# dan-lee-gh/monte-carlo-gp

Measured on AMD Instinct MI355X. Metric: race-simulations/sec (20 drivers, 60 laps), higher is better.
Workload: dtype f64

## Files before the change

monte_carlo_gp_amd/csrc/race_kernel_reg.hip.h:

```cpp
#pragma once
#include "race_common.hip.h"
#include "race_isa.hip.h"
#include "sort_networks.h"

#include <utility>

#ifndef MCGP_STAT
#define MCGP_STAT(what, value)
#endif
#ifndef MCGP_TRACE_PASS
#define MCGP_TRACE_PASS(sim, lap, pass, n_cand)
#endif
#ifndef MCGP_COOPERATIVE_EVENTS
#define MCGP_COOPERATIVE_EVENTS 1
#endif
#ifndef MCGP_GRID_EXACT
#define MCGP_GRID_EXACT 0
#endif
#ifndef MCGP_WIDE_EXACT
#define MCGP_WIDE_EXACT 0
#endif
#ifndef MCGP_WIDE_TIE_SHIFT
#define MCGP_WIDE_TIE_SHIFT 0
#endif

namespace mcgp {

constexpr uint32_t k3UsedMask = 7u;
constexpr uint32_t k3Drs = 1u << 3;
constexpr int k3IdShift = 4;
constexpr uint32_t k3IdMask = 31u << k3IdShift;
constexpr uint32_t k3Dnf = 1u << 9;
constexpr uint32_t k3SlotMask = k3IdMask | k3Dnf;
constexpr int k3CompShift = 10;
constexpr uint32_t k3CompMask = 7u << k3CompShift;
constexpr uint32_t k3Dirty = 1u << 13;
constexpr int k3AgeShift = 16;
constexpr uint32_t k3AgeMask = 0x7FFu << k3AgeShift;
constexpr int k3GposShift = 27;
__host__ __device__ constexpr uint32_t pk_driver16(uint32_t p) { return p & k3IdMask; }
__host__ __device__ constexpr uint32_t pk_slot16(uint32_t p) { return p & k3SlotMask; }
__host__ __device__ constexpr uint32_t pk_comp512(uint32_t p) { return (p & k3CompMask) >> (k3CompShift - 9); }
__host__ __device__ constexpr uint32_t pk_comp16(uint32_t p) { return (p >> (k3CompShift - 4)) & 0x70u; }
constexpr double kAgeFieldUnit = 1.0 / 65536.0;

constexpr size_t kLdsPerCu = 160 * 1024;
__host__ __device__ constexpr size_t align16(size_t x) { return (x + 15) / 16 * 16; }
constexpr int kWordRows = 8;
__host__ __device__ constexpr size_t per_thread_lds_bytes_reg(int n) { return (size_t)kWordRows * 4 + (size_t)n * 8; }
constexpr int kNumCompounds = 5;
__host__ __device__ constexpr size_t shared_lds_bytes_reg(int n)
{
    return (size_t)kNormalRows * 16 + (size_t)n * 16 + (size_t)(kMaxCars + n) * 16 +
           (size_t)((kNumCompounds - 1) * kMaxCars + n) * 16 + kCompStride * 16 + 64 + 128 + align16((size_t)n * n * 4) +
           align16((size_t)n * n * 8);
}
__host__ __device__ constexpr int reg_min_waves(int n) { return n <= 6 ? (n == 4 ? 4 : 6) : n <= 11 ? 4 : n <= 22 ? 3 : 2; }
constexpr int kMaxBlockWaves = 16;
constexpr size_t kLdsReserve = 256;
__host__ __device__ constexpr int block_shape_rank(int w) { return (w % 4 == 0 ? 0 : 100) + (w <= 8 ? 2 * (8 - w) : w - 8); }
__host__ __device__ constexpr int reg_block_waves(int n)
{
    const int cap = 4 * reg_min_waves(n);
    int best = 0, waves = 1;
    for (int w = 1; w <= kMaxBlockWaves; ++w) {
        int b = (int)((kLdsPerCu - kLdsReserve) / (shared_lds_bytes_reg(n) + (size_t)w * 64 * per_thread_lds_bytes_reg(n)));
        if (b * w > cap) b = cap / w;
        if (b < 1) continue;
        if (b * w > best || (b * w == best && block_shape_rank(w) < block_shape_rank(waves))) { best = b * w; waves = w; }
    }
    return waves;
}

__host__ __device__ constexpr size_t reg_retire_ws_bytes(int n, size_t lanes) { return (size_t)(n + 1) * lanes * 4; }

constexpr int kWideLdsRowsMax = 32 * 16;
constexpr int kNorm53LdsStride = 80;
__host__ __device__ constexpr size_t wide_fixed_lds_bytes(int n, int waves)
{
    return shared_lds_bytes_reg(n) - (size_t)kNormalRows * 16 + (size_t)waves * 64 * per_thread_lds_bytes_reg(n);
}
__host__ __device__ constexpr int wide_lds_rows(int n, int waves)
{
    const size_t fixed = wide_fixed_lds_bytes(n, waves);
    const size_t room = kLdsPerCu - kLdsReserve > fixed ? kLdsPerCu - kLdsReserve - fixed : 0;
    int rows = (int)(room / (size_t)kNorm53LdsStride) / 16 * 16;
    return rows > kWideLdsRowsMax ? kWideLdsRowsMax : rows;
}
__host__ __device__ constexpr size_t wide_lds_bytes(int n, int waves)
{
    return wide_fixed_lds_bytes(n, waves) + (size_t)wide_lds_rows(n, waves) * kNorm53LdsStride;
}
__host__ __device__ constexpr size_t wide_chain_bytes(int n, int total_laps)
{
    return total_laps >= 2 ? (size_t)(total_laps - 1) * (size_t)((n + 3) & ~3) * 8 : 0;
}
__host__ __device__ constexpr size_t wide_launch_lds_bytes(int n, int waves, int total_laps)
{
    const size_t base = wide_lds_bytes(n, waves), chain = wide_chain_bytes(n, total_laps);
    return base + chain + kLdsReserve <= kLdsPerCu ? base + chain : base;
}
template <int N, int WAVES = reg_block_waves(N), bool WIDE = false>
struct RegGeo {
    static constexpr int kWaves = WAVES;
    static constexpr bool kWide = WIDE;
    static constexpr int B = 64 * kWaves;
    static constexpr uint32_t oDrvA = 0;
    static constexpr uint32_t oDrvB = oDrvA + N * 16;
    static constexpr uint32_t oIc = oDrvB + (kMaxCars + N) * 16;
    static constexpr uint32_t oComp = oIc + ((kNumCompounds - 1) * kMaxCars + N) * 16;
    static constexpr uint32_t oDrs = oComp + kCompStride * 16;
    static constexpr uint32_t oPit = oDrs + 16;
    static constexpr uint32_t oDrsB = oDrs + 32;
    static constexpr uint32_t oLut = oDrsB + 32;
    static constexpr uint32_t oNorm = oLut + 128;
    static constexpr uint32_t oHist = oNorm + (WIDE ? 0 : kNormalRows * 16);
    static_assert(WIDE || oNorm >= kNormalRowBias * 16, "the inverse-normal rows are addressed through a base 48 rows before the table");
    static constexpr uint32_t oGrid = oHist + (uint32_t)align16((size_t)N * N * 4);
    static constexpr uint32_t oW = oGrid + (uint32_t)align16((size_t)N * N * 8);
    static constexpr uint32_t oLast = oW + (uint32_t)kWordRows * B * 4;
    static constexpr uint32_t oNorm53 = oLast + (uint32_t)N * B * 8;
    static constexpr int kNorm53Rows = WIDE ? wide_lds_rows(N, WAVES) : 0;
    static constexpr int kNorm53First = kNormal53Rows - kNorm53Rows;
    static constexpr uint32_t kBytes = oNorm53 + (uint32_t)kNorm53Rows * (uint32_t)kNorm53LdsStride;
    static constexpr uint32_t oChain = kBytes;
    static constexpr uint32_t kChainStride = (uint32_t)((N + 3) & ~3) * 8u;
    __host__ __device__ static constexpr bool chain_fits(int total_laps)
    {
        return WIDE && total_laps >= 2 && kBytes + wide_chain_bytes(N, total_laps) + kLdsReserve <= kLdsPerCu;
    }
    static_assert(oW == shared_lds_bytes_reg(N) - (WIDE ? (size_t)kNormalRows * 16 : 0) && oLast % 8 == 0, "LDS map");
    static_assert(oW % 16 == 0 && oNorm53 % 16 == 0, "the event handler parks fields with 16-byte LDS accesses (ds_write_b128 / ds_read_b128); table rows are read 16 bytes at a time");
    static_assert(kBytes == (WIDE ? wide_lds_bytes(N, WAVES) : per_thread_lds_bytes_reg(N) * B + shared_lds_bytes_reg(N)), "LDS map");
    static_assert(kBytes + kLdsReserve <= kLdsPerCu, "block does not fit LDS");
    static_assert(oLast < 65536, "row bases must fit the DS immediate offset");
};
constexpr int kWideMinLdsRows = 14 * 16;
__host__ __device__ constexpr int wide_block_waves(int n)
{
    if (n <= 22) {
        for (int w = 12; w > 8; --w)
            if (wide_fixed_lds_bytes(n, w) + kLdsReserve <= kLdsPerCu && wide_lds_rows(n, w) >= kWideMinLdsRows) return w;
    }
    int w = 8;
    while (w > 1 && wide_fixed_lds_bytes(n, w) + kLdsReserve > kLdsPerCu) --w;
    return w;
}
__host__ __device__ constexpr int wide_min_waves(int n) { return wide_block_waves(n) > 8 ? 3 : 2; }
template <int N>
using WideGeo = RegGeo<N, wide_block_waves(N), true>;

template <int N>
struct SortNetwork {
    int a[N * 8];
    int b[N * 8];
    int step[N * 8];
    int n;
    int ga[N * 8];
    int gn[N * 8];
    int n_groups;
    constexpr SortNetwork() : a{}, b{}, step{}, n(0), ga{}, gn{}, n_groups(0)
    {
        const SortNetworkTable *table = nullptr;
        for (const SortNetworkTable &t : kSortNetworks)
            if (t.n == N) table = &t;
        if (table) {
            for (int i = 0; i < table->size; ++i) {
                a[n] = table->pairs[i][0];
                b[n] = table->pairs[i][1];
                step[n] = table->pairs[i][2];
                ++n;
            }
        } else {
            int t = 0, s = 0;
            while ((1 << t) < N) ++t;
            for (int p = t > 0 ? 1 << (t - 1) : 0; p > 0; p >>= 1) {
                int q = 1 << (t - 1), r = 0, d = p;
                while (true) {
                    for (int i = 0; i < N - d; ++i)
                        if ((i & p) == r) { a[n] = i; b[n] = i + d; step[n] = s; ++n; }
                    ++s;
                    if (q == p) break;
                    d = q - p;
                    q >>= 1;
                    r = p;
                }
            }
        }
        for (int i = 0; i < n;) {
            const int len = (i + 1 < n && step[i + 1] == step[i]) ? 2 : 1;
            ga[n_groups] = i;
            gn[n_groups] = len;
            ++n_groups;
            i += len;
        }
    }
};

__device__ __forceinline__ bool cmpx(double &ca, uint32_t &pa, double &cb, uint32_t &pb)
{
    const bool sw = (ca > cb) || (ca == cb && pa > pb);
    double c0, c1;
// ... 146 lines not shown
    return strict;
}

template <int N, bool DISTINCT = false>
__device__ __forceinline__ void update_positions_reg(const double (&cum)[N], uint32_t (&pk)[N],
                                                     bool drs_allowed, double dirty_thr)
{
    bool first = true;
    double leader = 0.0, prev = 0.0;
#pragma unroll
    for (int i = 0; i < N; ++i) {
        const uint32_t p = pk[i];
        const bool act = !(p & k3Dnf);
        const double t = cum[i];
        leader = (act && first) ? t : leader;
        const double tbl = t - leader;
        const bool dirty = (DISTINCT ? !first : tbl > 0) && tbl < dirty_thr;
        const bool drs = !first && drs_allowed && (t - prev) < 1.0;
        pk[i] = (p & ~(k3Drs | k3Dirty)) | (dirty ? k3Dirty : 0u) | (drs ? k3Drs : 0u);
        prev = act ? t : prev;
        first = first && !act;
    }
}

__host__ __device__ constexpr int pit_regime(int remaining_laps)
{
    return remaining_laps > 30 ? 0 : remaining_laps > 20 ? 1 : remaining_laps > 15 ? 2 : 3;
}
__device__ __forceinline__ uint32_t pit_rule_word(int track, int regime, uint32_t used, uint32_t pop_sh, uint32_t pop_mh)
{
    const int remaining_laps = regime == 0 ? 31 : regime == 1 ? 21 : regime == 2 ? 16 : 0;
    uint32_t newc = stint_compound(track, remaining_laps);
    if (track == 0 && __popc(used) == 1 && ((used >> newc) & 1u)) {
        const uint32_t avail = 7u & ~used;
        const uint32_t popped = avail == 5u ? pop_sh : avail == 6u ? pop_mh : 0u;
        if (remaining_laps > 20) newc = (avail & 2u) ? 1u : popped;
        else newc = (avail & 1u) ? 0u : popped;
    }
    return (newc << k3CompShift) | ((used | (1u << newc)) & k3UsedMask);
}

constexpr double kRegTimeFloor = 8.0;
__host__ __device__ inline double reg_time_floor(const KParams &kp)
{
    const double z_max = kp.wide ? 8.5 : 6.5;
    double floor_ = __builtin_inf();
    double cdelta_min = __builtin_inf();
    for (int c = 0; c < 5; ++c) cdelta_min = kp.comp_delta[c] < cdelta_min ? kp.comp_delta[c] : cdelta_min;
    for (int d = 0; d < kp.n; ++d) {
        double eff_min = 0.0;
        for (int c = 0; c < 5; ++c) {
            const double e = kp.comp_deg[c] * kp.factor[d];
            eff_min = e < eff_min ? e : eff_min;
        }
        const double var = kp.variance[d] < 0 ? -kp.variance[d] : kp.variance[d];
        const double f = kp.base_pace[d] - var * z_max + eff_min * 2047.0;
        floor_ = f < floor_ ? f : floor_;
        if (!(f == f)) return f;
    }
    floor_ = floor_ + cdelta_min - 110.0 * 0.03 - (kp.drs_delta > 0 ? kp.drs_delta : 0.0) +
             (kp.dirty_pen < 0 ? kp.dirty_pen : 0.0) - 0.5 * 1.5 * z_max;
    return floor_;
}

__host__ __device__ inline bool reg_kernel_serves(const KParams &kp)
{
    if (!(kp.overtake_delta >= 0.0)) return false;
    const double big = 0x1p900, tiny = 0x1p-900;
    auto scalable = [&](double x) { return x == 0.0 || (x > -big && x < big && (x >= tiny || x <= -tiny)); };
    for (int d = 0; d < kp.n; ++d) {
        if (!scalable(kp.base_pace[d]) || !scalable(kp.tire_deg[d])) return false;
        for (int c = 0; c < 5; ++c)
            if (!scalable(kp.comp_deg[c] * kp.factor[d])) return false;
    }
    return reg_time_floor(kp) >= kRegTimeFloor;
}

template <int N, class G = RegGeo<N>>
__device__ __forceinline__ void reg_load_tables(const KParams *__restrict__ P, unsigned char *smem, uint32_t tid,
                                                const double *__restrict__ norm53 = nullptr)
{
    constexpr int B = G::B;
    uint32_t *s_hist = reinterpret_cast<uint32_t *>(smem + G::oHist);
    double *t_grid = reinterpret_cast<double *>(smem + G::oGrid);
    if constexpr (G::kWide) {
        double *t53 = reinterpret_cast<double *>(smem + G::oNorm53);
        for (uint32_t i = tid; i < (uint32_t)G::kNorm53Rows * 8u; i += B)
            t53[(i >> 3) * (kNorm53LdsStride / 8) + (i & 7u)] = norm53[(uint32_t)G::kNorm53First * 8u + i];
        if (G::chain_fits(P->total_laps)) {
            for (uint32_t d = tid; d < G::kChainStride / 8u; d += B) {
                const uint64_t q = d < (uint32_t)N ? P->q64_dnf[d] : 0ull;
                uint64_t S = q;
                for (int k = 2; k <= P->total_laps; ++k) {
                    *reinterpret_cast<uint64_t *>(smem + G::oChain + (uint32_t)(k - 2) * G::kChainStride + d * 8u) = S;
                    S = __umul64hi(S, q);
                }
            }
        }
    } else {
        float4 *t_norm = reinterpret_cast<float4 *>(smem + G::oNorm);
        for (uint32_t i = tid; i < (uint32_t)kNormalRows * 4; i += B)
            reinterpret_cast<uint32_t *>(t_norm)[i] = P->normal_bits[i];
    }
    for (uint32_t d = tid; d < (uint32_t)N; d += B) {
        double *a = reinterpret_cast<double *>(smem + G::oDrvA + d * 16);
        double *b = reinterpret_cast<double *>(smem + G::oDrvB + d * 16);
        const double qnan = __builtin_nan("");
        a[0] = P->variance[d];
        a[1] = P->base_pace[d];
        b[0] = P->base_pace[d] * 2147483648.0;
        b[1] = P->tire_deg[d] * 32768.0;
        b[2 * kMaxCars] = qnan;
        b[2 * kMaxCars + 1] = qnan;
    }
    if (tid < 2) {
        *reinterpret_cast<double *>(smem + G::oDrs + tid * k3Drs) = tid ? P->drs_delta : 0.0;
        *reinterpret_cast<double *>(smem + G::oDrsB + tid * k3Drs) = tid ? P->drs_delta * 2147483648.0 : 0.0;
        *reinterpret_cast<double *>(smem + G::oPit + tid * 8u) = tid ? P->pit_loss : 0.0;
    }
    for (uint32_t i = tid; i < (uint32_t)kNumCompounds * N; i += B) {
        const uint32_t c = i / N, d = i % N;
        unsigned char *r = smem + G::oIc + (c * kMaxCars + d) * 16;
        *reinterpret_cast<double *>(r) = (P->comp_deg[c] * P->factor[d]) * kAgeFieldUnit;
        *reinterpret_cast<uint32_t *>(r + 8) = (uint32_t)P->opt_laps[d * kCompStride + c] << 16;
        *reinterpret_cast<uint32_t *>(r + 12) = 0u;
    }
    for (uint32_t i = tid; i < 32u; i += B)
        *reinterpret_cast<uint32_t *>(smem + G::oLut + i * 4) =
            pit_rule_word(P->track, (int)(i >> 3), i & 7u, (uint32_t)P->pop_sh, (uint32_t)P->pop_mh);
    for (uint32_t c = tid; c < (uint32_t)kCompStride; c += B) {
        double *r = reinterpret_cast<double *>(smem + G::oComp + c * 16);
        r[0] = P->comp_delta[c];
        r[1] = 0.0;
    }
    for (uint32_t i = tid; i < (uint32_t)(N * N); i += B) {
        s_hist[i] = 0u;
        t_grid[(i % N) * N + (i / N)] = P->grid_probs[i];
    }
}

template <int N, class G = RegGeo<N>>
__device__ __forceinline__ void reg_flush_hist(unsigned char *smem, uint32_t tid, unsigned long long *__restrict__ hist)
{
    const uint32_t *s_hist = reinterpret_cast<const uint32_t *>(smem + G::oHist);
    for (uint32_t i = tid; i < (uint32_t)(N * N); i += G::B) {
        const uint32_t c = s_hist[i];
        if (c) atomicAdd(&hist[i], (unsigned long long)c);
    }
}

__device__ __forceinline__ uint32_t uniform_u32(uint32_t x)
{
#if defined(__HIP_DEVICE_COMPILE__)
    return (uint32_t)__builtin_amdgcn_readfirstlane((int)x);
#else
    return x;
#endif
}
template <int N, class G>
__device__ __forceinline__ uint32_t wide_pass_exact_body(const uint32_t (&pk)[N], double od31, uint32_t lap, uint32_t pass, uint32_t c0l,
                                                         uint32_t c1l, uint32_t k0l, uint32_t k1l, uint32_t tid)
{
    constexpr int B = G::B;
    const uint32_t tid4 = tid * 4u;
    auto w_row_ = [&](int r) -> uint32_t { return G::oW + (uint32_t)r * (B * 4) + tid4; };
    uint32_t hits53 = 0u;
    uint64_t thr64[N];
    uint32_t cand = 0u;
    {
        double pace_prev = 0.0;
#pragma unroll
        for (int i = 0; i < N; ++i) {
            const f64x2 bd = lds_ld_f64x2(G::oDrvB + pk_slot16(pk[i]));
            const double pace = bd.x + (double)(pk[i] & k3AgeMask) * bd.y;
            thr64[i] = 0ull;
            if (i > 0) {
                const double dl = (pace_prev - pace) + lds_ld<double>(G::oDrsB + (pk[i] & k3Drs));
                const bool c = dl > od31;
                double x = ceil_f64(dl * 0x1p21);
                x = x < 0x1p52 ? x : 0x1p52;
                const uint32_t xh = c ? cvt_u32_f64_sat(x * 0x1p-32) : 0u;
                const uint32_t xl = c ? cvt_u32_f64_sat(x - (double)xh * 0x1p32) : 0u;
                thr64[i] = ((uint64_t)xh << 32) | (uint64_t)xl;
                cand |= c ? (1u << i) : 0u;
            }
            pace_prev = pace;
        }
    }
    uint32_t rest = cand;
#pragma unroll 1
    for (int chunk = 0; MCGP_ANY(rest != 0u); ++chunk) {
        uint32_t m = rest;
#pragma unroll 1
        for (int k = 0; k < 4 && m != 0u; ++k) m &= m - 1u;
        const uint32_t cur = rest & ~m;
        uint32_t o0, o1, o2, o3;
        philox4x32_10(c0l, c1l, (uint32_t)lap, kPurposeOvt | (uint32_t)(8 * pass + chunk), k0l, k1l, o0, o1, o2, o3);
        lds_st<uint32_t>(w_row_(0), o0);
        lds_st<uint32_t>(w_row_(1), o1);
        lds_st<uint32_t>(w_row_(2), o2);
        lds_st<uint32_t>(w_row_(3), o3);
        philox4x32_10(c0l, c1l, (uint32_t)lap, kPurposeOvt | kCompanion | (uint32_t)(8 * pass + chunk), k0l, k1l, o0, o1, o2, o3);
        lds_st<uint32_t>(w_row_(4), o0);
        lds_st<uint32_t>(w_row_(5), o1);
        lds_st<uint32_t>(w_row_(6), o2);
        lds_st<uint32_t>(w_row_(7), o3);
        uint32_t h = 0u;
#pragma unroll
        for (int i = 1; i < N; ++i) {
            const uint32_t r = (uint32_t)__popc(cur & ((1u << i) - 1u)) * (uint32_t)(B * 4) + tid4;
            const uint64_t u = uniform53(lds_ld<uint32_t>(G::oW + r), lds_ld<uint32_t>(G::oW + (uint32_t)(4 * B * 4) + r));
            h |= u < thr64[i] ? (1u << i) : 0u;
        }
        hits53 |= h & cur;
        rest = m;
    }
    return hits53;
}
template <int N>
struct PkWords {
    uint32_t v[N];
};
template <int N, class G>
__device__ __attribute__((noinline)) uint32_t wide_pass_exact_fn(PkWords<N> field, double od31, uint32_t lap, uint32_t pass, uint32_t c0l,
                                                                 uint32_t c1l, uint32_t k0l_, uint32_t k1l_, uint32_t tid)
{
    return wide_pass_exact_body<N, G>(field.v, od31, lap, pass, c0l, c1l, uniform_u32(k0l_), uniform_u32(k1l_), tid);
}

template <int N, bool WIDE = false, class G = RegGeo<N>>
__device__ __forceinline__ void reg_simulate(const KParams *__restrict__ P, unsigned char *smem, uint32_t tid,
                                             uint32_t *__restrict__ ticket, uint64_t n_sims,
                                             uint64_t sim_offset, uint32_t seed_lo, uint32_t seed_hi,
                                             uint8_t *__restrict__ orders, const uint8_t *__restrict__ fixed_grid,
                                             uint32_t n_chunks, uint32_t *__restrict__ retire_ws_base, uint32_t ws_stride,
                                             uint32_t ws_first_lane, const double *__restrict__ norm53 = nullptr)
{
    constexpr int B = G::B;
    constexpr int kStepBatch = 4;
    constexpr bool kLean = WIDE && wide_min_waves(N) >= 3;
    constexpr int kPaceBatch = 5;
    static_assert(kStepBatch % 4 == 0, "a Philox block serves four consecutive places");
    const uint32_t tid4 = tid * 4u, tid8 = tid * 8u;
    const int L = P->total_laps;
    const int track = P->track;

    uint32_t *s_hist = reinterpret_cast<uint32_t *>(smem + G::oHist);

    auto w_row = [&](int r) -> uint32_t { return G::oW + (uint32_t)r * (B * 4) + tid4; };
    auto l_row = [&](int d) -> uint32_t { return G::oLast + (uint32_t)d * (B * 8) + tid8; };
    auto last_of = [&](uint32_t p) -> uint32_t { return ((p >> k3IdShift) & 31u) * (uint32_t)(B * 8) + tid8; };
    auto grid_byte = [&](int pos) -> uint32_t { return G::oW + (uint32_t)(pos >> 2) * (B * 4) + tid4 + (uint32_t)(pos & 3); };
    auto norm_row = [&](uint32_t off) -> float4 { return lds_ld_float4(G::oNorm - kNormalRowBias * 16u + off); };
    constexpr uint32_t kRareHi = (kNormal53HiBias + (uint32_t)(G::kNorm53First > 16 ? G::kNorm53First : 16)) << 16;
    [[maybe_unused]] auto norm53_row = [&](uint32_t hi, double (&c)[8]) {
        const uint32_t a = (hi >> 16) * (uint32_t)kNorm53LdsStride + (G::oNorm53 - (kNormal53HiBias + (uint32_t)G::kNorm53First) * (uint32_t)kNorm53LdsStride);
#pragma unroll
        for (int k = 0; k < 4; ++k) {
            const f64x2 v = lds_ld_f64x2(a + 16u * k);
            c[2 * k] = v.x;
            c[2 * k + 1] = v.y;
        }
    };
    [[maybe_unused]] auto normal53_one = [&](uint32_t w, uint32_t x) -> double {
        uint32_t hi;
        double t;
        normal53_prepare(w, x, hi, t);
        if (__builtin_expect(MCGP_ANY(G::kNorm53Rows == 0 || MCGP_WIDE_EXACT || hi < kRareHi), 0)) return normal53(w, x, norm53);
        double c[8];
        norm53_row(hi, c);
        return normal53_evaluate(w, c, t);
    };

    const double dirty_thr = P->dirty_thr;
    const float kNaN = __uint_as_float(0x7fc00000u);

    struct SlotIn {
        uint32_t pitw;
        double last, var, base, eff, cdelta, drs;
        uint32_t la;
        uint32_t fit;
    };
    auto load_slot = [&](uint32_t p, uint32_t lut_base) -> SlotIn {
        SlotIn r;
        r.fit = lds_ld<uint32_t>(((p & k3UsedMask) << 2) + lut_base);
        const uint32_t id16 = pk_driver16(p);
        r.la = id16 * (uint32_t)(B / 2) + tid8;
        r.last = lds_ld<double>(G::oLast + r.la);
        const uint32_t ic = id16 + pk_comp512(p);
        const f64x2 vb = lds_ld_f64x2(G::oDrvA + id16);
        r.var = vb.x;
        r.base = vb.y;
        uint32_t pad;
        lds_ld_f64_u32x2(G::oIc + ic, r.eff, r.pitw, pad);
        r.cdelta = lds_ld<double>(G::oComp + pk_comp16(p));
        r.drs = lds_ld<double>(G::oDrs + (p & k3Drs));
        return r;
    };

    for (uint32_t turn = 0u;; ++turn) {
        const uint32_t chunk = next_ticket(ticket, tid, turn, G::kWaves);
        if (chunk >= n_chunks) break;
        const uint64_t local = (uint64_t)chunk * 64ull + (uint64_t)(tid & 63u);
        const bool live = local < n_sims;
        if (!MCGP_ANY(live)) continue;
        const uint64_t sim = sim_offset + local;
        const uint32_t c0 = (uint32_t)sim, c1 = (uint32_t)(sim >> 32);

        double cum[N];
        uint32_t pk[N];

        {
            uint32_t remaining = (N >= 32) ? 0xffffffffu : ((1u << N) - 1u);
            int n_remaining = N;
            uint32_t g0 = 0, g1 = 0, g2 = 0, g3 = 0, h0 = 0, h1 = 0, h2 = 0, h3 = 0;
#pragma unroll 1
            for (int pos = 0; pos < N; ++pos) {
                uint32_t sel;
                if (fixed_grid) {
                    sel = fixed_grid[pos];
                } else {
                    if ((pos & 3) == 0) {
                        philox4x32_10(c0, c1, 0u, kPurposeGrid | (uint32_t)(pos >> 2), seed_lo, seed_hi, g0, g1, g2, g3);
                        if constexpr (WIDE)
                            philox4x32_10(c0, c1, 0u, kPurposeGrid | kCompanion | (uint32_t)(pos >> 2), seed_lo, seed_hi, h0, h1, h2, h3);
                    }
                    const uint32_t gw = (pos & 3) == 0 ? g0 : (pos & 3) == 1 ? g1 : (pos & 3) == 2 ? g2 : g3;
                    const uint32_t hw = (pos & 3) == 0 ? h0 : (pos & 3) == 1 ? h1 : (pos & 3) == 2 ? h2 : h3;
                    const double u = WIDE ? (double)uniform53(gw, hw) * 0x1p-53 : u32_to_unit(gw);
                    const uint32_t gcol = G::oGrid + (uint32_t)(pos * N) * 8u;
                    double acc = 0.0;
                    double A[N];
#pragma unroll
                    for (int d = 0; d < N; ++d) {
                        const double pd = ((remaining >> d) & 1u) ? lds_ld<double>(gcol + 8u * d) : 0.0;
                        acc = acc + pd;
                        A[d] = acc;
                    }
                    const double total = acc;
                    const double uc = u * total;
                    const double sure_gt = uc * (1.0 + 0x1p-40), sure_le = uc * (1.0 - 0x1p-40);
                    uint32_t n_le = 0u, n_le_lo = 0u;
#pragma unroll
                    for (int d = 0; d < N; ++d) {
                        n_le += A[d] > sure_gt ? 0u : 1u;
                        n_le_lo += A[d] > sure_le ? 0u : 1u;
                    }
                    const bool exact_path = MCGP_GRID_EXACT || !(total > 0x1p-900 && total < 0x1p900) || n_le != n_le_lo || n_le >= (uint32_t)N;
                    sel = n_le;
                    if (__builtin_expect(MCGP_ANY(exact_path), 0)) {
                        double p[N];
#pragma unroll
                        for (int d = 0; d < N; ++d) p[d] = ((remaining >> d) & 1u) ? lds_ld<double>(gcol + 8u * d) : 0.0;
                        const bool has_mass = total > 0;
                        const double uniform_p = 1.0 / (double)n_remaining;
                        double prob_sum = 0.0;
#pragma unroll
                        for (int d = 0; d < N; ++d) {
                            const double q = has_mass ? p[d] / total : uniform_p;
                            p[d] = ((remaining >> d) & 1u) ? q : 0.0;
                            prob_sum = prob_sum + p[d];
                        }
                        if (prob_sum > 0 && fabs(prob_sum - 1.0) > 1e-9) {
#pragma unroll
                            for (int d = 0; d < N; ++d) p[d] = p[d] / prob_sum;
                        }
                        double cdf = 0.0;
#pragma unroll
                        for (int d = 0; d < N; ++d) {
                            cdf = cdf + p[d];
                            p[d] = cdf;
                        }
                        const double cdf_last = cdf;
                        uint32_t above = 0u;
#pragma unroll
                        for (int d = 0; d < N; ++d) above |= !(p[d] / cdf_last <= u) ? (1u << d) : 0u;
                        const uint32_t sel_exact = above ? (uint32_t)__ffs((int)above) - 1u : 31u - (uint32_t)__clz((int)remaining);
                        sel = exact_path ? sel_exact : sel;
                    }
                }
                if ((remaining >> sel) & 1u) { remaining &= ~(1u << sel); --n_remaining; }
                lds_st<uint8_t>(grid_byte(pos), (uint8_t)sel);
            }
        }

#pragma unroll
        for (int i = 0; i < N; ++i) {
            const uint32_t id = lds_ld<uint8_t>(grid_byte(i));
            uint32_t comp, age;
            if (track == 2) { comp = 4u; age = 0u; }
            else if (track == 1) { comp = 3u; age = 0u; }
            else { comp = i < 10 ? 0u : 1u; age = i < 10 ? 4u : 0u; }
            pk[i] = (age << k3AgeShift) | (comp << k3CompShift) | ((1u << comp) & k3UsedMask) | (id << k3IdShift) |
                    ((uint32_t)i << k3GposShift);
            cum[i] = 0.0;
        }

        if constexpr (WIDE) {
#pragma unroll 1
            for (int d = 0; d < N; ++d) {
                uint32_t w0, w1, w2, w3, x0, x1, x2, x3;
                philox4x32_10(c0, c1, 1u, kPurposeCar | (uint32_t)d, seed_lo, seed_hi, w0, w1, w2, w3);
                philox4x32_10(c0, c1, 1u, kPurposeCar | kCompanion | (uint32_t)d, seed_lo, seed_hi, x0, x1, x2, x3);
                const bool out = uniform53(w0, x0) < P->t53_dnf1[d];
                lds_st<double>(l_row(d), out ? __builtin_nan("") : normal53_one(w1, x1));
            }
#pragma unroll
            for (int i = 0; i < N; ++i) {
                const uint32_t p = pk[i];
                const double z = lds_ld<double>(G::oLast + last_of(p));
                const uint32_t id16 = pk_driver16(p);
                const f64x2 vb = lds_ld_f64x2(G::oDrvA + id16);
                const double eff = lds_ld<double>(G::oIc + id16 + pk_comp512(p));
                const double cdelta = lds_ld<double>(G::oComp + pk_comp16(p));
                if (z != z) {
                    pk[i] = (p & ~k3AgeMask) | k3Dnf | (1u << k3AgeShift);
                    cum[i] = -(double)(i + 1) * 0x1p-1000;
                } else {
                    const double tire = (double)(p & k3AgeMask) * eff;
                    const double fuel_effect = (110.0 - 110.0) * 0.03;
                    const double noise = 0.0 + vb.x * z;
                    cum[i] = vb.y + tire - fuel_effect + cdelta - 0.0 + noise;
                }
            }
#pragma unroll 1
            for (int d = 0; d < N; ++d) {
                uint32_t w0, w1, w2, w3, x0, x1, x2, x3;
                philox4x32_10(c0, c1, 1u, kPurposeCar | (uint32_t)d, seed_lo, seed_hi, w0, w1, w2, w3);
                philox4x32_10(c0, c1, 1u, kPurposeCar | kCompanion | (uint32_t)d, seed_lo, seed_hi, x0, x1, x2, x3);
                lds_st<double>(l_row(d), normal53_one(w2, x2));
            }
#pragma unroll
            for (int i = 0; i < N; ++i) {
                const uint32_t p = pk[i];
                const double zs = lds_ld<double>(G::oLast + last_of(p));
                if (!(p & k3Dnf)) {
// ... 400 lines not shown
                                double zc[R][8];
#pragma unroll
                                for (int j = 0; j < R; ++j) norm53_row(zhi[j0 + j], zc[j]);
#pragma unroll
                                for (int j = 0; j < R; ++j)
                                    z[j0 + j] = (i0 + j0 + j < N) ? normal53_evaluate(w[(j0 + j) >> 2][(j0 + j) & 3], zc[j], zt[j0 + j]) : 0.0;
                            }
                        } else {
#pragma unroll
                            for (int j = 0; j < kStepBatch; ++j) {
                                z[j] = (i0 + j < N) ? normal53(w[j >> 2][j & 3], x[j >> 2][j & 3], norm53) : 0.0;
                                pin(z[j]);
                                sched_fence();
                            }
                        }
                        if constexpr (kLean) {
#pragma unroll
                            for (int j = 0; j < kStepBatch; ++j) pin(z[j]);
                            sched_fence();
#pragma unroll
                            for (int j = 0; j < kStepBatch; ++j)
                                if (i0 + j < N) in[j] = load_slot(pk[i0 + j], lut_base);
                        }
                    } else {
#pragma unroll
                        for (int j0 = 0; j0 < kStepBatch; j0 += 2) {
                            uint32_t zrow[2];
                            float zt[2];
                            float4 zc[2];
#pragma unroll
                            for (int j = 0; j < 2; ++j) normal_prepare(w[(j0 + j) >> 2][(j0 + j) & 3], zrow[j], zt[j]);
#pragma unroll
                            for (int j = 0; j < 2; ++j) zc[j] = norm_row(zrow[j]);
#pragma unroll
                            for (int j = 0; j < 2; ++j)
                                z[j0 + j] = (i0 + j0 + j < N) ? normal_evaluate(w[(j0 + j) >> 2][(j0 + j) & 3], zc[j], zt[j]) : 0.0f;
                        }
                    }
#pragma unroll
                    for (int j = 0; j < kStepBatch; ++j) {
                        const int i = i0 + j;
                        if (i >= N) continue;
                        const SlotIn &s = in[j];
                        const uint32_t p = pk[i];
                        const bool active = !(p & k3Dnf);
                        const bool dnf_hit = __double2hiint(s.last) < 0;
                        const bool run = active && !dnf_hit;
                        const double ahead_last = carry;
                        carry = active ? s.last : carry;
                        const uint32_t agef = p & k3AgeMask;
                        const double tire = (double)agef * s.eff;
                        const double drs_gain = s.drs;
                        const double noise = s.var * (double)z[j];
                        const double clean = s.base + tire - fuel_effect + s.cdelta - drs_gain + noise;
                        const uint32_t dirty_m = (uint32_t)((int32_t)(p << (31 - 13)) >> 31);
                        const double pen_if_dirty = __hiloint2double((int)((uint32_t)__double2hiint(dirty_pen_lap) & dirty_m),
                                                                     (int)((uint32_t)__double2loint(dirty_pen_lap) & dirty_m));
                        const double ahead_if_dirty = __hiloint2double((int)((uint32_t)__double2hiint(ahead_last) & dirty_m),
                                                                       (int)((uint32_t)__double2loint(ahead_last) & dirty_m));
                        const double lap_time = max_abs_f64(ahead_if_dirty, clean + pen_if_dirty);
                        const bool pit = run && pit_window && agef >= s.pitw;
                        const uint32_t p_pit = (p & ~(k3CompMask | k3UsedMask | k3AgeMask)) | s.fit;
                        uint32_t p_run = pit ? p_pit : p + (1u << k3AgeShift);
                        uint32_t p_ret = (p & ~k3AgeMask) | retire_word;
                        pin(p_run);
                        pin(p_ret);
                        const uint32_t p_act = dnf_hit ? p_ret : p_run;
                        pk[i] = active ? p_act : p;
                        const double lap_add = run ? lap_time : 0.0;
                        const double pit_add = lds_ld<double>(G::oPit + (pit ? 8u : 0u));
                        cum[i] = (cum[i] + lap_add) + pit_add;
                        pin(cum[i]);
                        lds_st<double>(G::oLast + s.la, lap_time);
                    }
                }
            }

            bool distinct_times = network_sort<N>(cum, pk);
#pragma unroll
            for (int pass = 0; pass < 3; ++pass) {
                uint32_t thr[N];
                uint32_t ow[N];
                uint32_t n_attempts = 0u;
                [[maybe_unused]] auto wide_pass_exact = [&]() -> uint32_t {
                    if constexpr (kLean) {
                        PkWords<N> f;
#pragma unroll
                        for (int i = 0; i < N; ++i) f.v[i] = pk[i];
                        return wide_pass_exact_fn<N, G>(f, od31, (uint32_t)lap, (uint32_t)pass, c0l, c1l, k0l, k1l, tid);
                    } else {
                        return wide_pass_exact_body<N, G>(pk, od31, (uint32_t)lap, (uint32_t)pass, c0l, c1l, k0l, k1l, tid);
                    }
                };
                {
                    {
                        uint32_t o0, o1, o2, o3;
                        philox4x32_10(c0l, c1l, (uint32_t)lap, kPurposeOvt | (uint32_t)(8 * pass), k0l, k1l, o0, o1, o2, o3);
                        lds_st<uint32_t>(w_row(0), o0);
                        lds_st<uint32_t>(w_row(1), o1);
                        lds_st<uint32_t>(w_row(2), o2);
                        lds_st<uint32_t>(w_row(3), o3);
                        philox4x32_10(c0l, c1l, (uint32_t)lap, kPurposeOvt | (uint32_t)(8 * pass + 1), k0l, k1l, o0, o1, o2, o3);
                        lds_st<uint32_t>(w_row(4), o0);
                        lds_st<uint32_t>(w_row(5), o1);
                        lds_st<uint32_t>(w_row(6), o2);
                        lds_st<uint32_t>(w_row(7), o3);
                    }
                    uint32_t row = tid4;
                    {
                        constexpr int H = kPaceBatch;
                            double pace_prev = 0.0;
#pragma unroll
                        for (int h = 0; h < N; h += H) {
                            sched_fence();
                            double pb[H], pd[H], pa[H];
#pragma unroll
                            for (int j = 0; j < H; ++j) {
                                if (h + j < N) {
                                    const uint32_t id16 = pk_slot16(pk[h + j]);
                                    const f64x2 bd = lds_ld_f64x2(G::oDrvB + id16);
                                    pb[j] = bd.x;
                                    pd[j] = bd.y;
                                    pa[j] = lds_ld<double>(G::oDrsB + (pk[h + j] & k3Drs));
                                }
                            }
#pragma unroll
                            for (int j = 0; j < H; ++j) {
                                const int i = h + j;
                                if (i < N) {
                                    const double pace = pb[j] + (double)(pk[i] & k3AgeMask) * pd[j];
                                    if (i > 0) {
                                        const double dl = (pace_prev - pace) + pa[j];
                                        uint32_t next;
                                        ovt_threshold<(uint32_t)(B * 4), !WIDE>(dl, od31, row, thr[i], next);
                                        ow[i] = lds_ld<uint32_t>(G::oW + row);
                                        row = next;
                                    }
                                    pace_prev = pace;
                                }
                            }
                        }
                        thr[0] = 0u;
                        ow[0] = 0u;
                    }
                    const uint32_t words_end = row - tid4;
                    MCGP_STAT(0 + pass, words_end != 0u);
                    if (words_end == 0u) break;
                    n_attempts = words_end / (uint32_t)(B * 4);
                    if constexpr (WIDE) {
                        bool tie = false;
#pragma unroll
                        for (int i = 1; i < N; ++i) tie |= ((ow[i] ^ thr[i]) >> MCGP_WIDE_TIE_SHIFT) == 0u;
                        MCGP_STAT(11, tie);
                        if (__builtin_expect(MCGP_ANY(tie || MCGP_WIDE_EXACT || words_end > (uint32_t)(kWordRows * B * 4)), 0)) {
                            const uint32_t hits = wide_pass_exact();
#pragma unroll
                            for (int i = 1; i < N; ++i) {
                                thr[i] = (hits >> i) & 1u;
                                ow[i] = 0u;
                            }
                        }
                    } else if (__builtin_expect(MCGP_ANY(words_end > (uint32_t)(kWordRows * B * 4)), 0)) {
                        uint32_t cand = 0u;
#pragma unroll
                        for (int i = 1; i < N; ++i) cand |= thr[i] != 0u ? (1u << i) : 0u;
                        uint32_t hits = 0u, rest = cand;
#pragma unroll 1
                        for (int chunk = 0; rest != 0u; ++chunk) {
                            uint32_t m = rest;
#pragma unroll 1
                            for (int k = 0; k < kWordRows && m != 0u; ++k) m &= m - 1u;
                            const uint32_t cur = rest & ~m;
#pragma unroll 1
                            for (int b = 0; b < 2; ++b) {
                                uint32_t o0, o1, o2, o3;
                                philox4x32_10(c0l, c1l, (uint32_t)lap, kPurposeOvt | (uint32_t)(8 * pass + 2 * chunk + b), k0l,
                                              k1l, o0, o1, o2, o3);
                                lds_st<uint32_t>(w_row(4 * b + 0), o0);
                                lds_st<uint32_t>(w_row(4 * b + 1), o1);
                                lds_st<uint32_t>(w_row(4 * b + 2), o2);
                                lds_st<uint32_t>(w_row(4 * b + 3), o3);
                            }
                            uint32_t h = 0u;
#pragma unroll
                            for (int i = 1; i < N; ++i) {
                                const uint32_t word = lds_ld<uint32_t>(G::oW + (uint32_t)__popc(cur & ((1u << i) - 1u)) * (uint32_t)(B * 4) + tid4);
                                h |= word < thr[i] ? (1u << i) : 0u;
                            }
                            hits |= h & cur;
                            rest = m;
                        }
#pragma unroll
                        for (int i = 1; i < N; ++i) {
                            thr[i] = (hits >> i) & 1u;
                            ow[i] = 0u;
                        }
                    }
                }
                bool any_succ = false;
#pragma unroll
                for (int i = 1; i < N; ++i) {
                    const bool hit = ow[i] < thr[i];
                    const double nb = cum[i - 1] - 0.1;
                    const double na = nb + 0.3;
                    cum[i] = hit ? nb : cum[i];
                    cum[i - 1] = hit ? na : cum[i - 1];
                    any_succ |= hit;
                }
                MCGP_STAT(4 + pass, any_succ);
                MCGP_STAT(8, n_attempts);
                MCGP_TRACE_PASS(local, lap, pass, (int)n_attempts);
                (void)n_attempts;
                if (!any_succ) break;
                distinct_times = resort_after_overtakes<N>(cum, pk);
            }
            if (!MCGP_ANY(!distinct_times))
                update_positions_reg<N, true>(cum, pk, lap > 2 && lap > drs_disabled_until, dirty_thr);
            else
                update_positions_reg<N>(cum, pk, lap > 2 && lap > drs_disabled_until, dirty_thr);
        }

        uint32_t key[N];
        {
            uint32_t g = 0u;
#pragma unroll
            for (int i = 0; i < N; ++i) {
                if (i > 0) g += cum[i] != cum[i - 1] ? 1u : 0u;
                const uint32_t p = pk[i];
                const uint32_t id = (p >> k3IdShift) & 31u;
                const uint32_t lapf = (p >> k3AgeShift) & 0x7FFu;
                const uint32_t key_dnf = (1u << 26) | ((2047u - lapf) << 15) | ((31u - g) << 10) | ((p >> k3GposShift) << 5) | id;
                const uint32_t key_run = ((uint32_t)i << 5) | id;
                key[i] = (p & k3Dnf) ? key_dnf : key_run;
            }
        }
        network_sort_keys<N>(key);
        if (live) {
#pragma unroll
// ... 114 lines not shown
```

Baseline: 148.2 million.

## Split pace table into base/deg/drs planes indexed by one packed offset

Rearranges the per-driver pace data into three separate LDS planes (base pace, degradation, DRS delta) that are all addressed by a single masked index taken from the packed driver word. This lets the compiler fold the three reads into ds_read2-style loads off one address and removes the separate DRS table lookup. It also drops the transposed starting-grid probability table from LDS and reads grid probabilities straight from global memory, which frees LDS and setup work. The cost is higher latency on the grid-sampling path, and the grid lookup now depends on caching.

```diff
diff --git a/monte_carlo_gp_amd/csrc/race_kernel_reg.hip.h b/monte_carlo_gp_amd/csrc/race_kernel_reg.hip.h
--- a/monte_carlo_gp_amd/csrc/race_kernel_reg.hip.h
+++ b/monte_carlo_gp_amd/csrc/race_kernel_reg.hip.h
@@ -39,7 +39,7 @@
 constexpr uint32_t k3AgeMask = 0x7FFu << k3AgeShift;
 constexpr int k3GposShift = 27;
 __host__ __device__ constexpr uint32_t pk_driver16(uint32_t p) { return p & k3IdMask; }
-__host__ __device__ constexpr uint32_t pk_slot16(uint32_t p) { return p & k3SlotMask; }
+__host__ __device__ constexpr uint32_t pk_pace(uint32_t p) { return p & (k3SlotMask | k3Drs); }
 __host__ __device__ constexpr uint32_t pk_comp512(uint32_t p) { return (p & k3CompMask) >> (k3CompShift - 9); }
 __host__ __device__ constexpr uint32_t pk_comp16(uint32_t p) { return (p >> (k3CompShift - 4)) & 0x70u; }
 constexpr double kAgeFieldUnit = 1.0 / 65536.0;
@@ -49,6 +49,16 @@
 constexpr int kWordRows = 8;
 __host__ __device__ constexpr size_t per_thread_lds_bytes_reg(int n) { return (size_t)kWordRows * 4 + (size_t)n * 8; }
 constexpr int kNumCompounds = 5;
+struct PaceOffsets {
+    uint32_t deg, drs, end;
+};
+__host__ __device__ constexpr PaceOffsets pace_table_offsets(int n)
+{
+    const uint32_t t = (uint32_t)(kMaxCars + n) * 16u;
+    if (n <= 10) return {16u * n, 32u * n, 512u + 48u * n};
+    if (n <= 16) return {16u * n, 512u + 32u * n, 512u + 32u * n + t};
+    return {t, 2 * t, 3 * t};
+}
 __host__ __device__ constexpr size_t shared_lds_bytes_reg(int n)
 {
     return (size_t)kNormalRows * 16 + (size_t)n * 16 + (size_t)(kMaxCars + n) * 16 +
@@ -102,22 +112,26 @@
 }
 template <int N, int WAVES = reg_block_waves(N), bool WIDE = false>
 struct RegGeo {
+    static constexpr PaceOffsets kPace = pace_table_offsets(N);
     static constexpr int kWaves = WAVES;
     static constexpr bool kWide = WIDE;
     static constexpr int B = 64 * kWaves;
-    static constexpr uint32_t oDrvA = 0;
-    static constexpr uint32_t oDrvB = oDrvA + N * 16;
-    static constexpr uint32_t oIc = oDrvB + (kMaxCars + N) * 16;
+    static constexpr uint32_t oPaceBase = 0;
+    static constexpr uint32_t oPaceDeg = kPace.deg;
+    static constexpr uint32_t oPaceDrs = kPace.drs;
+    static_assert(oPaceDeg / 8 < 256, "ds_read2_b64 offset");
+    static constexpr uint32_t oDrvA = (uint32_t)align16(kPace.end);
+    static constexpr uint32_t oIc = oDrvA + N * 16;
     static constexpr uint32_t oComp = oIc + ((kNumCompounds - 1) * kMaxCars + N) * 16;
     static constexpr uint32_t oDrs = oComp + kCompStride * 16;
     static constexpr uint32_t oPit = oDrs + 16;
-    static constexpr uint32_t oDrsB = oDrs + 32;
-    static constexpr uint32_t oLut = oDrsB + 32;
+    static constexpr uint32_t oLut = (oPit + 16 + 31) & ~31u;
     static constexpr uint32_t oNorm = oLut + 128;
     static constexpr uint32_t oHist = oNorm + (WIDE ? 0 : kNormalRows * 16);
     static_assert(WIDE || oNorm >= kNormalRowBias * 16, "the inverse-normal rows are addressed through a base 48 rows before the table");
-    static constexpr uint32_t oGrid = oHist + (uint32_t)align16((size_t)N * N * 4);
-    static constexpr uint32_t oW = oGrid + (uint32_t)align16((size_t)N * N * 8);
+    static constexpr uint32_t kTablesEnd = oHist + (uint32_t)align16((size_t)N * N * 4);
+    static_assert(kTablesEnd <= shared_lds_bytes_reg(N) - (WIDE ? (size_t)kNormalRows * 16 : 0), "the tables fit the block's shared bytes");
+    static constexpr uint32_t oW = (uint32_t)shared_lds_bytes_reg(N) - (WIDE ? (uint32_t)kNormalRows * 16 : 0u);
     static constexpr uint32_t oLast = oW + (uint32_t)kWordRows * B * 4;
     static constexpr uint32_t oNorm53 = oLast + (uint32_t)N * B * 8;
     static constexpr int kNorm53Rows = WIDE ? wide_lds_rows(N, WAVES) : 0;
@@ -430,7 +444,6 @@
 {
     constexpr int B = G::B;
     uint32_t *s_hist = reinterpret_cast<uint32_t *>(smem + G::oHist);
-    double *t_grid = reinterpret_cast<double *>(smem + G::oGrid);
     if constexpr (G::kWide) {
         double *t53 = reinterpret_cast<double *>(smem + G::oNorm53);
         for (uint32_t i = tid; i < (uint32_t)G::kNorm53Rows * 8u; i += B)
@@ -452,18 +465,19 @@
     }
     for (uint32_t d = tid; d < (uint32_t)N; d += B) {
         double *a = reinterpret_cast<double *>(smem + G::oDrvA + d * 16);
-        double *b = reinterpret_cast<double *>(smem + G::oDrvB + d * 16);
-        const double qnan = __builtin_nan("");
         a[0] = P->variance[d];
         a[1] = P->base_pace[d];
-        b[0] = P->base_pace[d] * 2147483648.0;
-        b[1] = P->tire_deg[d] * 32768.0;
-        b[2 * kMaxCars] = qnan;
-        b[2 * kMaxCars + 1] = qnan;
+    }
+    for (uint32_t i = tid; i < 4u * N; i += B) {
+        const uint32_t d = i >> 2, drs = i & 1u, retired = (i >> 1) & 1u;
+        const uint32_t e = (retired * kMaxCars + d) * 16u + drs * 8u;
+        const double qnan = __builtin_nan("");
+        *reinterpret_cast<double *>(smem + G::oPaceBase + e) = retired ? qnan : P->base_pace[d] * 2147483648.0;
+        *reinterpret_cast<double *>(smem + G::oPaceDeg + e) = retired ? qnan : P->tire_deg[d] * 32768.0;
+        *reinterpret_cast<double *>(smem + G::oPaceDrs + e) = drs ? P->drs_delta * 2147483648.0 : 0.0;
     }
     if (tid < 2) {
         *reinterpret_cast<double *>(smem + G::oDrs + tid * k3Drs) = tid ? P->drs_delta : 0.0;
-        *reinterpret_cast<double *>(smem + G::oDrsB + tid * k3Drs) = tid ? P->drs_delta * 2147483648.0 : 0.0;
         *reinterpret_cast<double *>(smem + G::oPit + tid * 8u) = tid ? P->pit_loss : 0.0;
     }
     for (uint32_t i = tid; i < (uint32_t)kNumCompounds * N; i += B) {
@@ -481,10 +495,7 @@
         r[0] = P->comp_delta[c];
         r[1] = 0.0;
     }
-    for (uint32_t i = tid; i < (uint32_t)(N * N); i += B) {
-        s_hist[i] = 0u;
-        t_grid[(i % N) * N + (i / N)] = P->grid_probs[i];
-    }
+    for (uint32_t i = tid; i < (uint32_t)(N * N); i += B) s_hist[i] = 0u;
 }
 
 template <int N, class G = RegGeo<N>>
@@ -519,11 +530,11 @@
         double pace_prev = 0.0;
 #pragma unroll
         for (int i = 0; i < N; ++i) {
-            const f64x2 bd = lds_ld_f64x2(G::oDrvB + pk_slot16(pk[i]));
-            const double pace = bd.x + (double)(pk[i] & k3AgeMask) * bd.y;
+            const uint32_t e = pk_pace(pk[i]);
+            const double pace = lds_ld<double>(G::oPaceBase + e) + (double)(pk[i] & k3AgeMask) * lds_ld<double>(G::oPaceDeg + e);
             thr64[i] = 0ull;
             if (i > 0) {
-                const double dl = (pace_prev - pace) + lds_ld<double>(G::oDrsB + (pk[i] & k3Drs));
+                const double dl = (pace_prev - pace) + lds_ld<double>(G::oPaceDrs + e);
                 const bool c = dl > od31;
                 double x = ceil_f64(dl * 0x1p21);
                 x = x < 0x1p52 ? x : 0x1p52;
@@ -676,12 +687,13 @@
                     const uint32_t gw = (pos & 3) == 0 ? g0 : (pos & 3) == 1 ? g1 : (pos & 3) == 2 ? g2 : g3;
                     const uint32_t hw = (pos & 3) == 0 ? h0 : (pos & 3) == 1 ? h1 : (pos & 3) == 2 ? h2 : h3;
                     const double u = WIDE ? (double)uniform53(gw, hw) * 0x1p-53 : u32_to_unit(gw);
-                    const uint32_t gcol = G::oGrid + (uint32_t)(pos * N) * 8u;
+                    const double *gcol = P->grid_probs + pos;
                     double acc = 0.0;
                     double A[N];
 #pragma unroll
                     for (int d = 0; d < N; ++d) {
-                        const double pd = ((remaining >> d) & 1u) ? lds_ld<double>(gcol + 8u * d) : 0.0;
+                        const double g = gcol[d * N];
+                        const double pd = ((remaining >> d) & 1u) ? g : 0.0;
                         acc = acc + pd;
                         A[d] = acc;
                     }
@@ -699,7 +711,10 @@
                     if (__builtin_expect(MCGP_ANY(exact_path), 0)) {
                         double p[N];
 #pragma unroll
-                        for (int d = 0; d < N; ++d) p[d] = ((remaining >> d) & 1u) ? lds_ld<double>(gcol + 8u * d) : 0.0;
+                        for (int d = 0; d < N; ++d) {
+                            const double g = gcol[d * N];
+                            p[d] = ((remaining >> d) & 1u) ? g : 0.0;
+                        }
                         const bool has_mass = total > 0;
                         const double uniform_p = 1.0 / (double)n_remaining;
                         double prob_sum = 0.0;
@@ -1301,11 +1316,10 @@
 #pragma unroll
                             for (int j = 0; j < H; ++j) {
                                 if (h + j < N) {
-                                    const uint32_t id16 = pk_slot16(pk[h + j]);
-                                    const f64x2 bd = lds_ld_f64x2(G::oDrvB + id16);
-                                    pb[j] = bd.x;
-                                    pd[j] = bd.y;
-                                    pa[j] = lds_ld<double>(G::oDrsB + (pk[h + j] & k3Drs));
+                                    const uint32_t e = pk_pace(pk[h + j]);
+                                    pb[j] = lds_ld<double>(G::oPaceBase + e);
+                                    pd[j] = lds_ld<double>(G::oPaceDeg + e);
+                                    pa[j] = lds_ld<double>(G::oPaceDrs + e);
                                 }
                             }
 #pragma unroll
```

After: 150.0 million (median of 6 runs). 1.01x the previous value.

## Rewrite wide exact overtake pass as a rolled, register-lean loop with lazy Philox

Applied to the files above, without the earlier changes.

The wide-mode exact overtake fallback is rewritten as a non-unrolled loop that rotates the packed driver array through pk[0], instead of keeping a per-driver 64-bit threshold array and regenerating Philox blocks into shared memory in chunks. It reuses the already-stored LDS words for the first kWordRows candidates and calls Philox only when a candidate index exceeds them or when the low 21 bits actually decide the comparison. The noinline wrapper and the readfirstlane uniformisation of the keys are removed, and the tie check is reduced to a single min over XORs. The aim is lower register pressure in the hot kernel and less RNG work on the rare exact path, at the cost of a serial per-driver loop and divergent lane-wise Philox calls.

```diff
diff --git a/monte_carlo_gp_amd/csrc/race_kernel_reg.hip.h b/monte_carlo_gp_amd/csrc/race_kernel_reg.hip.h
--- a/monte_carlo_gp_amd/csrc/race_kernel_reg.hip.h
+++ b/monte_carlo_gp_amd/csrc/race_kernel_reg.hip.h
@@ -497,83 +497,54 @@
     }
 }
 
-__device__ __forceinline__ uint32_t uniform_u32(uint32_t x)
-{
-#if defined(__HIP_DEVICE_COMPILE__)
-    return (uint32_t)__builtin_amdgcn_readfirstlane((int)x);
-#else
-    return x;
-#endif
-}
 template <int N, class G>
-__device__ __forceinline__ uint32_t wide_pass_exact_body(const uint32_t (&pk)[N], double od31, uint32_t lap, uint32_t pass, uint32_t c0l,
-                                                         uint32_t c1l, uint32_t k0l, uint32_t k1l, uint32_t tid)
+__device__ __forceinline__ uint32_t wide_pass_exact(uint32_t (&pk)[N], double od31, uint32_t lap, uint32_t pass, uint32_t c0l,
+                                                    uint32_t c1l, uint32_t k0l, uint32_t k1l, uint32_t tid)
 {
     constexpr int B = G::B;
     const uint32_t tid4 = tid * 4u;
-    auto w_row_ = [&](int r) -> uint32_t { return G::oW + (uint32_t)r * (B * 4) + tid4; };
-    uint32_t hits53 = 0u;
-    uint64_t thr64[N];
-    uint32_t cand = 0u;
-    {
-        double pace_prev = 0.0;
-#pragma unroll
-        for (int i = 0; i < N; ++i) {
-            const f64x2 bd = lds_ld_f64x2(G::oDrvB + pk_slot16(pk[i]));
-            const double pace = bd.x + (double)(pk[i] & k3AgeMask) * bd.y;
-            thr64[i] = 0ull;
-            if (i > 0) {
-                const double dl = (pace_prev - pace) + lds_ld<double>(G::oDrsB + (pk[i] & k3Drs));
-                const bool c = dl > od31;
-                double x = ceil_f64(dl * 0x1p21);
-                x = x < 0x1p52 ? x : 0x1p52;
-                const uint32_t xh = c ? cvt_u32_f64_sat(x * 0x1p-32) : 0u;
-                const uint32_t xl = c ? cvt_u32_f64_sat(x - (double)xh * 0x1p32) : 0u;
-                thr64[i] = ((uint64_t)xh << 32) | (uint64_t)xl;
-                cand |= c ? (1u << i) : 0u;
-            }
-            pace_prev = pace;
+    auto word_of = [](uint32_t k, uint32_t o0, uint32_t o1, uint32_t o2, uint32_t o3) -> uint32_t {
+        const uint32_t lo = (k & 1u) ? o1 : o0, hi = (k & 1u) ? o3 : o2;
+        return (k & 2u) ? hi : lo;
+    };
+    uint32_t hits = 0u, k = 0u;
+    double pace_prev = 0.0;
+#pragma unroll 1
+    for (uint32_t i = 0u; i < (uint32_t)N; ++i) {
+        const uint32_t p = pk[0];
+        const f64x2 bd = lds_ld_f64x2(G::oDrvB + pk_slot16(p));
+        const double pace = bd.x + (double)(p & k3AgeMask) * bd.y;
+        if (i > 0u) {
+            const double dl = (pace_prev - pace) + lds_ld<double>(G::oDrsB + (p & k3Drs));
+            const bool c = dl > od31;
+            double x = ceil_f64(dl * 0x1p21);
+            x = x < 0x1p52 ? x : 0x1p52;
+            const uint32_t xh = c ? cvt_u32_f64_sat(x * 0x1p-32) : 0u;
+            const uint32_t xl = c ? cvt_u32_f64_sat(x - (double)xh * 0x1p32) : 0u;
+            const uint64_t T = ((uint64_t)xh << 32) | (uint64_t)xl;
+            const uint32_t blk = kPurposeOvt | (8u * pass + (k >> 2));
+            uint32_t w = lds_ld<uint32_t>(G::oW + (k < (uint32_t)kWordRows ? k : 0u) * (uint32_t)(B * 4) + tid4);
+            if (MCGP_ANY(c && k >= (uint32_t)kWordRows)) {
+                uint32_t o0, o1, o2, o3;
+                philox4x32_10(c0l, c1l, lap, blk, k0l, k1l, o0, o1, o2, o3);
+                w = k < (uint32_t)kWordRows ? w : word_of(k, o0, o1, o2, o3);
+            }
+            bool hit = uniform53(w, 0u) < T;
+            const bool open = c && (MCGP_WIDE_EXACT || hit != (uniform53(w, 0xFFFFFFFFu) < T));
+            if (MCGP_ANY(open)) {
+                uint32_t o0, o1, o2, o3;
+                philox4x32_10(c0l, c1l, lap, blk | kCompanion, k0l, k1l, o0, o1, o2, o3);
+                hit = open ? uniform53(w, word_of(k, o0, o1, o2, o3)) < T : hit;
+            }
+            hits |= (c && hit) ? (1u << i) : 0u;
+            k += c ? 1u : 0u;
         }
-    }
-    uint32_t rest = cand;
-#pragma unroll 1
-    for (int chunk = 0; MCGP_ANY(rest != 0u); ++chunk) {
-        uint32_t m = rest;
-#pragma unroll 1
-        for (int k = 0; k < 4 && m != 0u; ++k) m &= m - 1u;
-        const uint32_t cur = rest & ~m;
-        uint32_t o0, o1, o2, o3;
-        philox4x32_10(c0l, c1l, (uint32_t)lap, kPurposeOvt | (uint32_t)(8 * pass + chunk), k0l, k1l, o0, o1, o2, o3);
-        lds_st<uint32_t>(w_row_(0), o0);
-        lds_st<uint32_t>(w_row_(1), o1);
-        lds_st<uint32_t>(w_row_(2), o2);
-        lds_st<uint32_t>(w_row_(3), o3);
-        philox4x32_10(c0l, c1l, (uint32_t)lap, kPurposeOvt | kCompanion | (uint32_t)(8 * pass + chunk), k0l, k1l, o0, o1, o2, o3);
-        lds_st<uint32_t>(w_row_(4), o0);
-        lds_st<uint32_t>(w_row_(5), o1);
-        lds_st<uint32_t>(w_row_(6), o2);
-        lds_st<uint32_t>(w_row_(7), o3);
-        uint32_t h = 0u;
-#pragma unroll
-        for (int i = 1; i < N; ++i) {
-            const uint32_t r = (uint32_t)__popc(cur & ((1u << i) - 1u)) * (uint32_t)(B * 4) + tid4;
-            const uint64_t u = uniform53(lds_ld<uint32_t>(G::oW + r), lds_ld<uint32_t>(G::oW + (uint32_t)(4 * B * 4) + r));
-            h |= u < thr64[i] ? (1u << i) : 0u;
-        }
-        hits53 |= h & cur;
-        rest = m;
-    }
-    return hits53;
-}
-template <int N>
-struct PkWords {
-    uint32_t v[N];
-};
-template <int N, class G>
-__device__ __attribute__((noinline)) uint32_t wide_pass_exact_fn(PkWords<N> field, double od31, uint32_t lap, uint32_t pass, uint32_t c0l,
-                                                                 uint32_t c1l, uint32_t k0l_, uint32_t k1l_, uint32_t tid)
-{
-    return wide_pass_exact_body<N, G>(field.v, od31, lap, pass, c0l, c1l, uniform_u32(k0l_), uniform_u32(k1l_), tid);
+        pace_prev = pace;
+#pragma unroll
+        for (int j = 0; j + 1 < N; ++j) pk[j] = pk[j + 1];
+        pk[N - 1] = p;
+    }
+    return hits;
 }
 
 template <int N, bool WIDE = false, class G = RegGeo<N>>
@@ -1266,16 +1237,6 @@
                 uint32_t thr[N];
                 uint32_t ow[N];
                 uint32_t n_attempts = 0u;
-                [[maybe_unused]] auto wide_pass_exact = [&]() -> uint32_t {
-                    if constexpr (kLean) {
-                        PkWords<N> f;
-#pragma unroll
-                        for (int i = 0; i < N; ++i) f.v[i] = pk[i];
-                        return wide_pass_exact_fn<N, G>(f, od31, (uint32_t)lap, (uint32_t)pass, c0l, c1l, k0l, k1l, tid);
-                    } else {
-                        return wide_pass_exact_body<N, G>(pk, od31, (uint32_t)lap, (uint32_t)pass, c0l, c1l, k0l, k1l, tid);
-                    }
-                };
                 {
                     {
                         uint32_t o0, o1, o2, o3;
@@ -1332,12 +1293,13 @@
                     if (words_end == 0u) break;
                     n_attempts = words_end / (uint32_t)(B * 4);
                     if constexpr (WIDE) {
-                        bool tie = false;
-#pragma unroll
-                        for (int i = 1; i < N; ++i) tie |= ((ow[i] ^ thr[i]) >> MCGP_WIDE_TIE_SHIFT) == 0u;
+                        uint32_t m = 0xFFFFFFFFu;
+#pragma unroll
+                        for (int i = 1; i < N; ++i) { const uint32_t d = ow[i] ^ thr[i]; m = d < m ? d : m; }
+                        const bool tie = (m >> MCGP_WIDE_TIE_SHIFT) == 0u;
                         MCGP_STAT(11, tie);
                         if (__builtin_expect(MCGP_ANY(tie || MCGP_WIDE_EXACT || words_end > (uint32_t)(kWordRows * B * 4)), 0)) {
-                            const uint32_t hits = wide_pass_exact();
+                            const uint32_t hits = wide_pass_exact<N, G>(pk, od31, (uint32_t)lap, (uint32_t)pass, c0l, c1l, k0l, k1l, tid);
 #pragma unroll
                             for (int i = 1; i < N; ++i) {
                                 thr[i] = (hits >> i) & 1u;
```

Result: no change. 148.5 million before, 148.6 million after, median of 6 (+0.0%).
